# caki35/UNet-Torch

Measured on AMD Instinct MI355X. Metric: images/sec training step, 4-level U-Net 1ch→2cls 512×512, at 1/2/4/8 MI355X, higher is better.
Workload: dtype f16

## Files before the change

### unet-torch_amd/csrc/conv_mfma.hip

```cpp
#include "kernels.h"
#include <stdlib.h>

typedef _Float16 half8 __attribute__((ext_vector_type(8)));
typedef _Float16 half4 __attribute__((ext_vector_type(4)));
typedef float floatx16 __attribute__((ext_vector_type(16)));

#ifdef UMI_STAMP
__device__ unsigned long long umi_stamp_buf[2048 * 8];
#define UMI_T(var)                                                                        \
    unsigned long long var;                                                               \
    __builtin_amdgcn_sched_barrier(0);                                                    \
    asm volatile("s_memtime %0\n\ts_waitcnt lgkmcnt(0)" : "=s"(var)::"memory");           \
    __builtin_amdgcn_sched_barrier(0)
extern "C" int umi_debug_read_stamps(void* dst) {
    return (int)hipMemcpyFromSymbol(dst, HIP_SYMBOL(umi_stamp_buf), sizeof(umi_stamp_buf));
}
#endif

namespace {

constexpr int HALO_W = 34;
constexpr int ROWB = 48;

template <int TH, int BN, int SC = 1, bool K32 = false>
struct Cfg {
    static_assert(!K32 || SC == 2, "K32 stages 32-channel halo tiles");
    static constexpr int WN = BN / 64;
    static constexpr int WM = 4 / WN;
    static_assert(TH / WM == 4, "every wave owns 4 image rows");
    static constexpr int HALO_PIX = (TH + 2) * HALO_W;
    static constexpr int NQ = 2 * SC;
    static constexpr int HROWB = NQ * 16 + 16;
    static constexpr int HPASS = 256 / NQ;
    static constexpr int HB = HALO_PIX * HROWB;
    static constexpr int WROWB = K32 ? 64 : ROWB;
    static constexpr int WSTG = 3 * BN * 64;
    static constexpr int WB = K32 ? 2 * WSTG : 9 * BN * ROWB;
    static constexpr int P = TH * 32;
    static constexpr int ERS = BN * 2 + 16;
    static constexpr int EB = P * ERS;
    static constexpr int SMEM = (HB + WB) > EB ? (HB + WB) : EB;
    static constexpr int KPH = (HALO_PIX + HPASS - 1) / HPASS;
    static constexpr int NPW = K32 ? 3 * BN * 4 : 9 * BN * 2;
    static constexpr int KPW = (NPW + 255) / 256;
    static constexpr int TSTEP = 128 / BN;
    static constexpr bool W_LAST_PARTIAL = !K32 && (KPW - 1) * TSTEP + (TSTEP - 1) >= 9;
    static constexpr int WCO = BN / 32, WRW = 4 / WCO;
    static_assert(!K32 || TH == 8 * WRW, "K32: every wave owns 8 image rows");
    static constexpr int PRE = SC == 2 ? 6 : 8;
};

struct BnRed { const half_t* y; int ld; const float4* tx; const float* rstd; };

__device__ __forceinline__ void* umi_uniform_ptr(const void* p) {
    const unsigned long a = (unsigned long)p;
    const unsigned lo = __builtin_amdgcn_readfirstlane((unsigned)a), hi = __builtin_amdgcn_readfirstlane((unsigned)(a >> 32));
    return (void*)(((unsigned long)hi << 32) | lo);
}

struct Tile { int n, ty0, tx0, c0, cvalid, pt; };

template <int TH, int BN, int SC, bool K32, bool HAS_TX, int EPI>
__global__ __launch_bounds__(256, 2) void conv3x3_mfma_kernel(
    const half_t* __restrict__ x, int ldx, const float4* __restrict__ tx, const half_t* __restrict__ wp8,
    half_t* __restrict__ y, int ldy, float* __restrict__ part, int N, int H, int W, int Ci, int Co, int tiles_x,
    int tiles_y, int n_co, int xcd_chunk, BnRed bn) {
    using C = Cfg<TH, BN, SC, K32>;
    constexpr int HROWB = C::HROWB;
    __shared__ __attribute__((aligned(16))) unsigned char smem[C::SMEM];
    __shared__ float4 txbuf[2][16 * SC];

    const int tid = threadIdx.x;
    const int lane = tid & 63;
    const int wave = tid >> 6;
    const int wn = wave % C::WN, wm = wave / C::WN;
#ifdef UMI_STAMP
    UMI_T(t_start);
    unsigned long long seg[5] = {0, 0, 0, 0, 0}, t_epi = 0, t_pro = 0, eps[4] = {0, 0, 0, 0};
    unsigned n_chunks_done = 0;
#endif

    const int q = (tid >> 3) & 1;
    const int srow = ((tid >> 4) << 3) | (tid & 7);
    const int hq = SC == 1 ? q : (tid >> 3) & (C::NQ - 1);
    const int hrow = SC == 1 ? srow : ((tid >> 5) << 3) | (tid & 7);

    const int tap0 = srow / BN, wcol = srow % BN;
    const int Ci8 = Ci >> 3;
    const int wstep_s = __builtin_amdgcn_readfirstlane(C::TSTEP * Ci8 * Co * 16);
    const int wl_base = C::HB + srow * ROWB + q * 16;
    const bool w_last_ok = tap0 + (C::KPW - 1) * C::TSTEP < 9;
    const int wl_last = w_last_ok ? wl_base + (C::KPW - 1) * 128 * ROWB : C::HB + srow * ROWB + 32;

    const int lrow = lane & 31, lhalf = lane >> 5;
    const int b_base = ((wm * 4) * HALO_W + lrow) * HROWB + lhalf * 16;
    const int a_base = C::HB + (wn * 64 + lrow) * ROWB + lhalf * 16;
    const int wc = wave % C::WCO, wr = wave / C::WCO;
    const int l16 = lane & 15, lg = lane >> 4;
    const int bk_base = ((wr * 8) * HALO_W + l16) * HROWB + lg * 16;
    const int ak_base = C::HB + (wc * 32 + l16) * C::WROWB + ((lg ^ ((l16 >> 1) & 3)) * 16);
    const int wkl_base = C::HB + (((tid >> 5) << 3) | (tid & 7)) * C::WROWB + ((((tid >> 3) & 3) ^ ((tid >> 1) & 3)) * 16);
    const int wdy_s = __builtin_amdgcn_readfirstlane(3 * Ci8 * Co * 16);
    const int nchunks = Ci >> 4;

    constexpr unsigned OOB = 0x7FFFFFFFu;
    constexpr unsigned WBAD = 0x40000000u;
    unsigned hoff[C::KPH];
    int hl_a, hl_b, hl_last;
    unsigned wbase_v, wbase_l;
    __amdgpu_buffer_rsrc_t xrs, wrs;

    auto decode = [&](int item) {
        int wid = item;
        if (xcd_chunk > 0 && wid < 8 * xcd_chunk) wid = (wid & 7) * xcd_chunk + (wid >> 3);
        Tile t;
        const int cb = wid % n_co;
        t.pt = wid / n_co;
        t.n = t.pt / (tiles_x * tiles_y);
        const int rem = t.pt - t.n * tiles_x * tiles_y;
        t.ty0 = (rem / tiles_x) * TH;
        t.tx0 = (rem % tiles_x) * 32;
        t.c0 = cb * BN;
        t.cvalid = Co - t.c0 < BN ? Co - t.c0 : BN;
        return t;
    };
#define UMI_PLAN(t_)                                                                                                   \
    do {                                                                                                              \
        int tid_ = threadIdx.x;                                                                                       \
        asm volatile("" : "+v"(tid_));                                                                                \
        const int q = (tid_ >> 3) & 1, srow = ((tid_ >> 4) << 3) | (tid_ & 7);                                        \
        const int hq = SC == 1 ? q : (tid_ >> 3) & (C::NQ - 1), hrow = SC == 1 ? srow : ((tid_ >> 5) << 3) | (tid_ & 7); \
        const int tap0 = srow / BN, wcol = srow % BN;                                                                 \
        const unsigned wbase = (unsigned)(((tap0 * (Ci >> 3) + q) * Co + wcol) * 16);                                 \
        const bool w_last_ok = tap0 + (C::KPW - 1) * C::TSTEP < 9;                                                    \
        _Pragma("unroll") for (int k = 0; k < C::KPH; ++k) {                                                          \
                                 \
            const int hp = hrow + C::HPASS * k;                                                                       \
            const int hy = hp / HALO_W, hx = hp - hy * HALO_W;                                                        \
            const int gy = (t_).ty0 + hy - 1, gx = (t_).tx0 + hx - 1;                                                 \
            const bool inimg = (hp < C::HALO_PIX) && gy >= 0 && gy < H && gx >= 0 && gx < W;                          \
            hoff[k] = inimg ? (unsigned)(gy * W + gx) * (unsigned)(ldx * 2) + hq * 16 : OOB;                          \
            const int hpc = hp < C::HALO_PIX ? hp : C::HALO_PIX - 1;                                                  \
            if (k == C::KPH - 1) hl_last = inimg ? hp * HROWB + hq * 16 : hpc * HROWB + C::NQ * 16;                   \
        }                                                                                                             \
        hl_a = hrow * HROWB + hq * 16;                                                                                \
        hl_b = hrow * HROWB + C::NQ * 16;                                                                             \
        xrs = __builtin_amdgcn_make_buffer_rsrc(umi_uniform_ptr(x + (long)(t_).n * H * W * ldx), 0,                   \
                                                (int)((long)H * W * ldx * 2), 0x00020000);                            \
        wrs = __builtin_amdgcn_make_buffer_rsrc(umi_uniform_ptr(wp8 + (long)(t_).c0 * 8), 0,                          \
                                                (int)((long)9 * Ci * Co * 2 - (long)(t_).c0 * 16), 0x00020000);       \
        const bool wok = wcol < (t_).cvalid;                                   \
        wbase_v = wok ? wbase : WBAD;                                                                                 \
        wbase_l = (wok && w_last_ok) ? wbase : WBAD;                                                                  \
        if constexpr (K32) {        \
            const int wrow_ = ((tid_ >> 5) << 3) | (tid_ & 7), wq_ = (tid_ >> 3) & 3;                                 \
            const unsigned wb_ = (unsigned)((wq_ * Co + wrow_) * 16);                                                 \
            wbase_v = wrow_ < (t_).cvalid ? wb_ : WBAD;                                                               \
            wbase_l = wrow_ + 64 < (t_).cvalid ? wb_ + 64 * 16 : WBAD;                                                \
        }                                                                                                             \
    } while (0)
#define UMI_ZERO_PADDING()                                                                                             \
    do {                                                                                                              \
        int tid_ = threadIdx.x;                                                                                       \
        asm volatile("" : "+v"(tid_));                                                                                \
        const int hq = SC == 1 ? (tid_ >> 3) & 1 : (tid_ >> 3) & (C::NQ - 1);                                         \
        const int hrow = SC == 1 ? ((tid_ >> 4) << 3) | (tid_ & 7) : ((tid_ >> 5) << 3) | (tid_ & 7);                 \
        _Pragma("unroll") for (int k = 0; k < C::KPH; ++k) {                                                          \
            const int hp = hrow + C::HPASS * k;                                                                       \
            if (hp < C::HALO_PIX && hoff[k] == OOB) {                                                                 \
                unsigned z0 = 0;                                                                                      \
                asm volatile("" : "+v"(z0));         \
                *reinterpret_cast<uint4*>(smem + hp * HROWB + hq * 16) = make_uint4(z0, z0, z0, z0);                  \
            }                                                                                                         \
        }                                                                                                             \
    } while (0)

    half8 hraw[C::KPH], wraw[C::KPW];
#define UMI_ISSUE_H(sc_)                                                                                          \
    do {                                                                                                          \
        _Pragma("unroll") for (int k = 0; k < C::KPH; ++k)                                                        \
            hraw[k] = __builtin_bit_cast(half8, __builtin_amdgcn_raw_buffer_load_b128(xrs, hoff[k], (sc_) * (32 * SC), 0)); \
    } while (0)
#define UMI_ISSUE_W(c_)                                                                                           \
    do {                                                                                                          \
        _Pragma("unroll") for (int k = 0; k < C::KPW; ++k)                                                        \
            wraw[k] = __builtin_bit_cast(half8, __builtin_amdgcn_raw_buffer_load_b128(                            \
                wrs, (C::W_LAST_PARTIAL && k == C::KPW - 1) ? wbase_l : wbase_v, (c_) * 2 * Co * 16 + k * wstep_s, 0)); \
    } while (0)

#define UMI_ISSUE_WK(sc_, dx_)                                                                                    \
    do {                                                                                                          \
        const int ws_ = (((dx_) * Ci8 + 4 * (sc_)) * Co) * 16;                                                    \
        _Pragma("unroll") for (int k = 0; k < C::KPW; ++k)                                                        \
            wraw[k] = __builtin_bit_cast(half8, __builtin_amdgcn_raw_buffer_load_b128(                            \
                wrs, (BN == 128 && (k & 1)) ? wbase_l : wbase_v, ws_ + (BN == 128 ? k >> 1 : k) * wdy_s, 0));     \
    } while (0)

    const bool tx_wave = __builtin_amdgcn_readfirstlane(tid >> 6) == 0;
    const int txi = lane & (16 * SC - 1);
    const int txs = (txi & 7) * C::NQ + (txi >> 3);
    const int nsc = nchunks / SC;
    float4 txr = make_float4(0.f, 1.f, 0.f, 0.f);
    int txc = 0;
    const __amdgpu_buffer_rsrc_t txrs = __builtin_amdgcn_make_buffer_rsrc(umi_uniform_ptr(tx), 0, HAS_TX ? Ci * 16 : 0, 0x00020000);
#define UMI_TX_ROWS(sc_) __builtin_bit_cast(float4, __builtin_amdgcn_raw_buffer_load_b128(txrs, txi * 16, (sc_) * (16 * SC * 16), 0))

    const Tile cur = decode(blockIdx.x);
    UMI_PLAN(cur);
    UMI_ISSUE_H(0);
    half8 wraw1[K32 ? C::KPW : 1];
    if constexpr (K32) {
        UMI_ISSUE_WK(0, 0);
#pragma unroll
        for (int k = 0; k < C::KPW; ++k)
            wraw1[k] = __builtin_bit_cast(half8, __builtin_amdgcn_raw_buffer_load_b128(
                wrs, (BN == 128 && (k & 1)) ? wbase_l : wbase_v, Ci8 * Co * 16 + (BN == 128 ? k >> 1 : k) * wdy_s, 0));
    } else UMI_ISSUE_W(0);
    UMI_ZERO_PADDING();
    if (HAS_TX) {
        if (tx_wave) {
            txbuf[0][txs] = UMI_TX_ROWS(0);
            txbuf[1][txs] = UMI_TX_ROWS(1 % nsc);
            txc = 2 % nsc;
            txr = UMI_TX_ROWS(txc);
        }
        __syncthreads();
    }
    {
        typedef float floatx4 __attribute__((ext_vector_type(4)));
        floatx16 acc[2][4];
        floatx4 acck[2][16];
        if constexpr (K32) {
#pragma unroll
            for (int a = 0; a < 2; ++a)
#pragma unroll
                for (int b = 0; b < 16; ++b)
#pragma unroll
                    for (int r = 0; r < 4; ++r) acck[a][b][r] = 0.f;
        } else {
#pragma unroll
            for (int a = 0; a < 2; ++a)
#pragma unroll
                for (int b = 0; b < 4; ++b)
#pragma unroll
                    for (int r = 0; r < 16; ++r) acc[a][b][r] = 0.f;
        }
#ifdef UMI_STAMP
        UMI_T(t_loop);
        if (n_chunks_done == 0) t_pro = t_loop - t_start;
#endif
        if constexpr (!K32) {
        for (int ci_ = 0; ci_ < nchunks; ++ci_) {
            const int sci = ci_ / SC, sub = ci_ % SC;
            const bool first = SC == 1 || sub == 0;
#ifdef UMI_STAMP
            UMI_T(t0);
            asm volatile("s_waitcnt vmcnt(0)" ::: "memory");
            UMI_T(t0b);
#endif
            if (first) {
                if (HAS_TX) {
                    float4 t[8];
#pragma unroll
                    for (int j = 0; j < 8; ++j) t[j] = txbuf[sci & 1][j * C::NQ + hq];
#pragma unroll
                    for (int k = 0; k < C::KPH; ++k) hraw[k] = umi_tx8(hraw[k], t);
                }
#pragma unroll
                for (int k = 0; k < C::KPH; ++k)
                    *reinterpret_cast<half8*>(smem + (k == C::KPH - 1 ? hl_last : (hoff[k] != OOB ? hl_a : hl_b) + k * C::HPASS * HROWB)) = hraw[k];
            }
#pragma unroll
            for (int k = 0; k < C::KPW; ++k)
                *reinterpret_cast<half8*>(smem + ((C::W_LAST_PARTIAL && k == C::KPW - 1) ? wl_last : wl_base + k * 128 * ROWB)) = wraw[k];
#ifdef UMI_STAMP
            UMI_T(t1);
#endif
            __syncthreads();
#ifdef UMI_STAMP
            UMI_T(t2);
#endif
            if (first) {
                if (HAS_TX && tx_wave) {
                    txbuf[sci & 1][txs] = txr;
                    txc = txc + 1 < nsc ? txc + 1 : 0;
                    txr = UMI_TX_ROWS(txc);
                }
                if (sci + 1 < nsc) UMI_ISSUE_H(sci + 1);
            }
            if (ci_ + 1 < nchunks) UMI_ISSUE_W(ci_ + 1);

            __builtin_amdgcn_s_setprio(3);
#pragma unroll
            for (int dx = 0; dx < 3; ++dx) {
                half8 bf[6];
#pragma unroll
                for (int rr = 0; rr < 6; ++rr)
                    bf[rr] = *reinterpret_cast<const half8*>(smem + b_base + (rr * HALO_W + dx) * HROWB + sub * 32);
#pragma unroll
                for (int dy = 0; dy < 3; ++dy) {
                    half8 af[2];
#pragma unroll
                    for (int mt = 0; mt < 2; ++mt)
                        af[mt] = *reinterpret_cast<const half8*>(smem + a_base + ((dy * 3 + dx) * BN + mt * 32) * ROWB);
#pragma unroll
                    for (int mt = 0; mt < 2; ++mt)
#pragma unroll
                        for (int nt = 0; nt < 4; ++nt)
                            acc[mt][nt] = __builtin_amdgcn_mfma_f32_32x32x16_f16(af[mt], bf[nt + dy], acc[mt][nt], 0, 0, 0);
                }
            }
            constexpr int MPR = 2;
            __builtin_amdgcn_sched_group_barrier(0x100, C::PRE, 0);
#pragma unroll
            for (int i_ = 0; i_ < 36 - C::PRE; ++i_) {
                __builtin_amdgcn_sched_group_barrier(0x008, MPR, 0);
                __builtin_amdgcn_sched_group_barrier(0x100, 1, 0);
            }
            __builtin_amdgcn_sched_group_barrier(0x008, 36 * MPR - MPR * (36 - C::PRE), 0);
            __builtin_amdgcn_s_setprio(0);
#ifdef UMI_STAMP
            UMI_T(t3);
#endif
            __syncthreads();
#ifdef UMI_STAMP
            UMI_T(t4);
            seg[0] += t0b - t0; seg[1] += t1 - t0b; seg[2] += t2 - t1; seg[3] += t3 - t2; seg[4] += t4 - t3;
            ++n_chunks_done;
#endif
        }
        } else {
#pragma unroll
        for (int k = 0; k < C::KPW; ++k) *reinterpret_cast<half8*>(smem + wkl_base + k * 64 * C::WROWB) = wraw[k];
#pragma unroll
        for (int k = 0; k < C::KPW; ++k) wraw[k] = wraw1[k];
        int sci = 0, dx = 0, wcur = 0;
        const int nst = 3 * nsc;
        for (int st = 0; st < nst; ++st) {
            const bool first = dx == 0;
#ifdef UMI_STAMP
            UMI_T(t0);
            asm volatile("s_waitcnt vmcnt(0)" ::: "memory");
            UMI_T(t0b);
#endif
            if (first) {
#ifndef UMI_X_NOTX
                if (HAS_TX) {
                    float4 t[8];
#pragma unroll
                    for (int j = 0; j < 8; ++j) t[j] = txbuf[sci & 1][j * C::NQ + hq];
#pragma unroll
                    for (int k = 0; k < C::KPH; ++k) hraw[k] = umi_tx8(hraw[k], t);
                }
#endif
#ifdef UMI_X_NOHW
#pragma unroll
                for (int k = 0; k < C::KPH; ++k) asm volatile("" ::"v"(hraw[k]));
#else
#pragma unroll
                for (int k = 0; k < C::KPH; ++k)
                    *reinterpret_cast<half8*>(smem + (k == C::KPH - 1 ? hl_last : (hoff[k] != OOB ? hl_a : hl_b) + k * C::HPASS * HROWB)) = hraw[k];
#endif
            }
#ifdef UMI_STAMP
            UMI_T(t1);
#endif
            if (first) __syncthreads();
#ifdef UMI_STAMP
            UMI_T(t2);
#endif
            if (first) {
                if (HAS_TX && tx_wave) {
                    txbuf[sci & 1][txs] = txr;
                    txc = txc + 1 < nsc ? txc + 1 : 0;
                    txr = UMI_TX_ROWS(txc);
                }
                if (sci + 1 < nsc) UMI_ISSUE_H(sci + 1);
            }
            __builtin_amdgcn_s_setprio(3);
            {
                half8 af[3][2];
                const unsigned char* ap = smem + ak_base + wcur;
#pragma unroll
                for (int dy = 0; dy < 3; ++dy)
#pragma unroll
                    for (int ct = 0; ct < 2; ++ct)
                        af[dy][ct] = *reinterpret_cast<const half8*>(ap + (dy * BN + ct * 16) * C::WROWB);
                const unsigned char* bp = smem + bk_base + dx * HROWB;
#pragma unroll
                for (int hr = 0; hr < 10; ++hr)
#pragma unroll
                    for (int h = 0; h < 2; ++h) {
                        const half8 bf = *reinterpret_cast<const half8*>(bp + (hr * HALO_W + h * 16) * HROWB);
#pragma unroll
                        for (int dy = 0; dy < 3; ++dy) {
                            const int r = hr - dy;
                            if (r >= 0 && r < 8) {
#pragma unroll
                                for (int ct = 0; ct < 2; ++ct)
                                    acck[ct][r * 2 + h] = __builtin_amdgcn_mfma_f32_16x16x32_f16(af[dy][ct], bf, acck[ct][r * 2 + h], 0, 0, 0);
                            }
                        }
                    }
            }
            {
#ifdef UMI_X_NOWWRITE
#pragma unroll
                for (int k = 0; k < C::KPW; ++k) asm volatile("" ::"v"(wraw[k]));
#else
#pragma unroll
                for (int k = 0; k < C::KPW; ++k)
                    *reinterpret_cast<half8*>(smem + wkl_base + (C::WSTG - wcur) + k * 64 * C::WROWB) = wraw[k];
#endif
#ifndef UMI_X_NOWLOAD
                const int ndx = dx == 0 ? 2 : dx - 1;
                int nsci = dx == 0 ? sci : sci + 1;
                nsci = nsci < nsc ? nsci : nsc - 1;
                UMI_ISSUE_WK(nsci, ndx);
#endif
            }
#define UMI_G(n_) __builtin_amdgcn_sched_group_barrier(0x008, n_, 0); __builtin_amdgcn_sched_group_barrier(0x100, 1, 0)
            __builtin_amdgcn_sched_group_barrier(0x100, 10, 0);
            UMI_G(2); UMI_G(2); UMI_G(4); UMI_G(4);
            UMI_G(6); UMI_G(6); UMI_G(6); UMI_G(6); UMI_G(6); UMI_G(6); UMI_G(6); UMI_G(6); UMI_G(6); UMI_G(6); UMI_G(6); UMI_G(6);
#pragma unroll
            for (int i_ = 0; i_ < C::KPW; ++i_) {
                __builtin_amdgcn_sched_group_barrier(0x008, 1, 0);
                __builtin_amdgcn_sched_group_barrier(0x200, 1, 0);
            }
#pragma unroll
            for (int i_ = 0; i_ < C::KPW; ++i_) {
                __builtin_amdgcn_sched_group_barrier(0x008, (12 - C::KPW) / C::KPW, 0);
                __builtin_amdgcn_sched_group_barrier(0x020, 1, 0);
            }
#undef UMI_G
            __builtin_amdgcn_s_setprio(0);
#ifdef UMI_STAMP
            UMI_T(t3);
#endif
            __syncthreads();
#ifdef UMI_STAMP
            UMI_T(t4);
            seg[0] += t0b - t0; seg[1] += t1 - t0b; seg[2] += t2 - t1; seg[3] += t3 - t2; seg[4] += t4 - t3;
            ++n_chunks_done;
#endif
            wcur = C::WSTG - wcur;
            if (++dx == 3) { dx = 0; ++sci; }
        }
        }
#ifdef UMI_STAMP
        UMI_T(t_ep0);
#endif

        const int n = cur.n, ty0 = cur.ty0, tx0 = cur.tx0, c0 = cur.c0, cvalid = cur.cvalid, pt = cur.pt;
        if constexpr (K32) {
#pragma unroll
            for (int ct = 0; ct < 2; ++ct) {
                const int co = wc * 32 + ct * 16 + lg * 4;
                float4 ot[4];
                if (EPI == 3) {
#pragma unroll
                    for (int j = 0; j < 4; ++j)
                        ot[j] = co + j < cvalid ? bn.tx[c0 + co + j] : make_float4(0.f, 1.f, 0.f, 0.f);
                }
#pragma unroll
                for (int pt_ = 0; pt_ < 16; ++pt_) {
                    const int pix = (wr * 8 + (pt_ >> 1)) * 32 + (pt_ & 1) * 16 + l16;
                    half4 h;
#pragma unroll
                    for (int j = 0; j < 4; ++j) {
                        float v = acck[ct][pt_][j];
                        if (EPI == 3) v = umi_tx(v, ot[j]);
                        h[j] = (half_t)v;
                    }
                    *reinterpret_cast<half4*>(smem + pix * C::ERS + co * 2) = h;
                }
            }
        } else
#pragma unroll
        for (int mt = 0; mt < 2; ++mt)
#pragma unroll
            for (int g = 0; g < 4; ++g) {
                const int co = wn * 64 + mt * 32 + g * 8 + lhalf * 4;
                float4 ot[4];
                if (EPI == 3) {
#pragma unroll
                    for (int j = 0; j < 4; ++j)
                        ot[j] = co + j < cvalid ? bn.tx[c0 + co + j] : make_float4(0.f, 1.f, 0.f, 0.f);
                }
#pragma unroll
                for (int nt = 0; nt < 4; ++nt) {
                    const int pix = (wm * 4 + nt) * 32 + lrow;
                    half4 h;
#pragma unroll
                    for (int j = 0; j < 4; ++j) {
                        float v = acc[mt][nt][g * 4 + j];
                        if (EPI == 3) v = umi_tx(v, ot[j]);
                        h[j] = (half_t)v;
                    }
                    *reinterpret_cast<half4*>(smem + pix * C::ERS + co * 2) = h;
                }
            }
        __syncthreads();
#ifdef UMI_STAMP
        UMI_T(t_e1);
        eps[0] += t_e1 - t_ep0;
#endif

        constexpr int PPR = BN / 8;
        constexpr int PSTEP = 256 / PPR;
        constexpr int NK = C::P / PSTEP;
        const bool full_tile = (ty0 + TH <= H) && (tx0 + 32 <= W);
        constexpr int SL = PSTEP;
        const int cg = tid % PPR, sl = tid / PPR;
        float s[8], s2[8];
#pragma unroll
        for (int jj = 0; jj < 8; ++jj) s[jj] = s2[jj] = 0.f;
        {
            const int j = cg, p0 = sl;
            const unsigned char* sbase = smem + p0 * C::ERS + j * 16;
            const bool col_ok = j * 8 < cvalid;
            float4 t[8];
            float rs_[8];
            if (EPI == 2 && col_ok) {
#pragma unroll
                for (int jj = 0; jj < 8; ++jj) { t[jj] = bn.tx[c0 + j * 8 + jj]; rs_[jj] = bn.rstd[c0 + j * 8 + jj]; }
            }
#define UMI_EPI_REDUCE(v_, yv_)                                                                                        \
            do {                                                                                                      \
                if (EPI == 1) {                                                                                       \
                    const half8 hv = __builtin_bit_cast(half8, v_);                                                   \
                    _Pragma("unroll") for (int jj = 0; jj < 8; ++jj) { float f = (float)hv[jj]; s[jj] += f; s2[jj] = fmaf(f, f, s2[jj]); } \
                } else if (EPI == 2) {                                                                                \
                    const half8 hv = __builtin_bit_cast(half8, v_);                                                   \
                    _Pragma("unroll") for (int jj = 0; jj < 8; ++jj) {                                                \
                        const float yy = (float)(yv_)[jj];                                                            \
                        const float dz = umi_tx_pre(yy, t[jj]) > t[jj].w ? (float)hv[jj] : 0.f;                       \
                        s[jj] += dz;                                                                                  \
                        s2[jj] = fmaf(dz, (yy - t[jj].x) * rs_[jj], s2[jj]);                                          \
                    }                                                                                                 \
                }                                                                                                     \
            } while (0)
            const bool whole = __builtin_amdgcn_readfirstlane((int)(full_tile && cvalid == BN)) != 0;
            const long tile_pix = ((long)n * H + ty0) * W + tx0;
            half_t* ybase = y + tile_pix * ldy + c0 + j * 8;
            half8 yv[NK];
            if (EPI == 2 && whole) {
                const __amdgpu_buffer_rsrc_t brs = __builtin_amdgcn_make_buffer_rsrc(umi_uniform_ptr(bn.y + tile_pix * bn.ld + c0), 0, 0x7FFFF000, 0x00020000);
                const unsigned bvo = (unsigned)(p0 * bn.ld + j * 8) * 2u;
#pragma unroll
                for (int k = 0; k < NK; ++k)
                    yv[k] = __builtin_bit_cast(half8, __builtin_amdgcn_raw_buffer_load_b128(
                        brs, bvo, ((((k * PSTEP) >> 5) * W + ((k * PSTEP) & 31)) * bn.ld) * 2, 0));
            }
#ifdef UMI_STAMP
            UMI_T(t_e2);
            eps[1] += t_e2 - t_e1;
#endif
            if (whole) {
                const __amdgpu_buffer_rsrc_t yrs = __builtin_amdgcn_make_buffer_rsrc(umi_uniform_ptr(y + tile_pix * ldy + c0), 0, 0x7FFFF000, 0x00020000);
                const unsigned yvo = (unsigned)(p0 * ldy + j * 8) * 2u;
#pragma unroll
                for (int k = 0; k < NK; ++k) {
                    const uint4 v = *reinterpret_cast<const uint4*>(sbase + k * PSTEP * C::ERS);
                    typedef unsigned u32x4_t __attribute__((__vector_size__(4 * sizeof(unsigned))));
                    const u32x4_t vv = __builtin_bit_cast(u32x4_t, v);
                    __builtin_amdgcn_raw_buffer_store_b128(vv, yrs, yvo, ((((k * PSTEP) >> 5) * W + ((k * PSTEP) & 31)) * ldy) * 2, 0);
                    asm volatile("s_nop 1" ::"v"(vv));
                    UMI_EPI_REDUCE(v, yv[k]);
                }
            } else {
                const half_t* yb = EPI == 2 ? bn.y + tile_pix * bn.ld + c0 + j * 8 : nullptr;
#pragma unroll 8
                for (int k = 0; k < NK; ++k) {
                    const int p = p0 + k * PSTEP;
                    const int row = p >> 5, col = p & 31;
                    if (col_ok && (full_tile || (ty0 + row < H && tx0 + col < W))) {
                        const uint4 v = *reinterpret_cast<const uint4*>(sbase + k * PSTEP * C::ERS);
                        *reinterpret_cast<uint4*>(ybase + ((long)row * W + col) * ldy) = v;
                        half8 yv1;
                        if (EPI == 2) yv1 = *reinterpret_cast<const half8*>(yb + ((long)row * W + col) * bn.ld);
                        UMI_EPI_REDUCE(v, yv1);
                    }
                }
            }
#undef UMI_EPI_REDUCE
#ifdef UMI_STAMP
            UMI_T(t_e3);
            eps[2] += t_e3 - t_e2;
#endif
        }

        if (EPI == 1 || EPI == 2) {
            __syncthreads();
            float* rs = reinterpret_cast<float*>(smem);
#pragma unroll
            for (int j = 0; j < 8; ++j) {
                rs[(0 * SL + sl) * BN + cg * 8 + j] = s[j];
                rs[(1 * SL + sl) * BN + cg * 8 + j] = s2[j];
            }
            __syncthreads();
            if (tid < 2 * BN) {
                const int which = tid / BN, cc = tid % BN;
                float a = 0.f;
#pragma unroll 8
                for (int k = 0; k < SL; ++k) a += rs[(which * SL + k) * BN + cc];
                if (cc < cvalid) part[((long)pt * 2 + which) * Co + c0 + cc] = a;
            }
        }
#ifdef UMI_STAMP
        UMI_T(t_end);
        t_epi += t_end - t_ep0;
#endif
    }
#ifdef UMI_STAMP
    if (lane == 0 && blockIdx.x < 512) {
#pragma unroll
        for (int i = 0; i < 5; ++i) umi_stamp_buf[(blockIdx.x * 4 + wave) * 8 + i] = seg[i];
        umi_stamp_buf[(blockIdx.x * 4 + wave) * 8 + 5] = n_chunks_done;
        umi_stamp_buf[(blockIdx.x * 4 + wave) * 8 + 6] = t_pro;
#ifdef UMI_STAMP_EPI
        for (int i = 0; i < 3; ++i) umi_stamp_buf[(blockIdx.x * 4 + wave) * 8 + i] = eps[i];
#endif
        umi_stamp_buf[(blockIdx.x * 4 + wave) * 8 + 7] = t_epi * (unsigned long long)nchunks / (n_chunks_done ? n_chunks_done : 1);
    }
#endif
}

template <int TH, int BN, int SC, bool K32 = false>
int launch(const void* x, int ldx, const void* tx, const void* wp8, void* y, int ldy, float* part, int N, int H, int W,
           int Ci, int Co, const BnRed* bnred, hipStream_t s, const void* out_tx = nullptr) {
    const int tiles_x = (W + 31) / 32, tiles_y = (H + TH - 1) / TH, n_co = (Co + BN - 1) / BN;
    const long nblk = (long)N * tiles_x * tiles_y * n_co;
    if (nblk >= (1L << 31)) return UMI_ERR_UNSUPPORTED;
    dim3 grid((unsigned)nblk), block(256);
    static const bool xcd_off = [] { const char* e = getenv("UMI_CONV_NO_XCD_ORDER"); return e && e[0] == '1'; }();
    const int xcd_chunk = (n_co > 1 && !xcd_off) ? (int)(nblk / 8) : 0;
    const BnRed bn = bnred ? *bnred : BnRed{nullptr, 0, (const float4*)out_tx, nullptr};
#define GO(HT, EP)                                                                                               \
    hipLaunchKernelGGL((conv3x3_mfma_kernel<TH, BN, SC, K32, HT, EP>), grid, block, 0, s, (const half_t*)x, ldx, \
                       (const float4*)tx, (const half_t*)wp8, (half_t*)y, ldy, part, N, H, W, Ci, Co, tiles_x,   \
                       tiles_y, n_co, xcd_chunk, bn)
    if (out_tx) { if (tx) GO(true, 3); else GO(false, 3); }
    else if (bnred) { if (tx) GO(true, 2); else GO(false, 2); }
    else if (tx) { if (part) GO(true, 1); else GO(true, 0); }
    else    { if (part) GO(false, 1); else GO(false, 0); }
#undef GO
    UMI_LAUNCH_CHECK();
    return UMI_OK;
}

#undef UMI_ISSUE_H
#undef UMI_TX_ROWS
#undef UMI_ISSUE_W
#undef UMI_ISSUE_WK
#undef UMI_PLAN
#undef UMI_ZERO_PADDING
}

bool umi_conv3x3_mfma_ok(const ConvFwdProblem& p) {
    if (p.flags & (UMI_CONV_UPSAMPLE2 | UMI_CONV_FORCE_GENERIC)) return false;
    if (p.in_dtype != UMI_F16 || p.out_dtype != UMI_F16 || p.has_bias) return false;
    if (p.R != 3 || p.S != 3 || p.stride != 1 || p.pad != 1 || p.Ho != p.H || p.Wo != p.W) return false;
    if (p.Ci % 16 || p.Co % 8 || p.ldx % 8 || p.ldy % 8) return false;
    if ((long)p.N * p.H * p.W * (long)(p.ldx > p.ldy ? p.ldx : p.ldy) >= (1L << 40)) return false;
    return true;
}

#ifdef UMI_FORCE_BN64
static bool use_bn128(int Co) { (void)Co; return false; }
#else
static bool use_bn128(int Co) { return Co % 128 == 0; }
#endif

static int g_impl = [] { const char* e = getenv("UMI_CONV3X3_IMPL"); return e ? atoi(e) : 1; }();
extern "C" int umi_tune_conv3x3_impl(int impl) {
    const int old = g_impl;
    if (impl >= 1 && impl <= 8) g_impl = impl;
    return old;
}

static int pick_th(int Co) { return use_bn128(Co) ? 8 : 16; }

int umi_conv3x3_mfma_stat_rows(int N, int H, int W, int Co) {
    const int th = pick_th(Co);
    return N * ((W + 31) / 32) * ((H + th - 1) / th);
}

#define UMI_GO(x, tx, wp8, y, part, ...)                                                     \
    do {                                                                                     \
        const int Ci = p.Ci, Co = p.Co;                                                      \
        if (use_bn128(Co) && Ci % 32 == 0 && g_impl != 2)                                    \
            return launch<8, 128, 2, true>(x, p.ldx, tx, wp8, y, p.ldy, part, p.N, p.H, p.W, Ci, Co, __VA_ARGS__); \
        if (use_bn128(Co)) return launch<8, 128, 1>(x, p.ldx, tx, wp8, y, p.ldy, part, p.N, p.H, p.W, Ci, Co, __VA_ARGS__); \
        if (Ci % 32 == 0 && g_impl == 3)                                                     \
            return launch<16, 64, 2, true>(x, p.ldx, tx, wp8, y, p.ldy, part, p.N, p.H, p.W, Ci, Co, __VA_ARGS__); \
        if (Ci % 32 == 0 && g_impl != 2)                                                     \
            return launch<16, 64, 2>(x, p.ldx, tx, wp8, y, p.ldy, part, p.N, p.H, p.W, Ci, Co, __VA_ARGS__); \
        return launch<16, 64, 1>(x, p.ldx, tx, wp8, y, p.ldy, part, p.N, p.H, p.W, Ci, Co, __VA_ARGS__); \
    } while (0)

int umi_conv3x3_mfma(const ConvFwdProblem& p, const void* x, const void* tx, const void* wp8, void* y, float* stat_part,
                     hipStream_t s) {
    UMI_GO(x, tx, wp8, y, stat_part, nullptr, s);
}

int umi_conv3x3_mfma_bnred(const ConvFwdProblem& p, const void* dy, const void* wp8, void* da, const void* ybn, int ldybn,
                           const void* txbn, const float* rstd, float* part, hipStream_t s) {
    const BnRed bn{(const half_t*)ybn, ldybn, (const float4*)txbn, rstd};
    UMI_GO(dy, nullptr, wp8, da, part, &bn, s);
}

int umi_conv3x3_mfma_act(const ConvFwdProblem& p, const void* x, const void* tx, const void* wp8, const void* out_tx, void* y,
                         hipStream_t s) {
    UMI_GO(x, tx, wp8, y, nullptr, nullptr, s, out_tx);
}
#undef UMI_GO
```

Baseline: 748.3.

## Prefetch epilogue bn.y residual tile into idle halo/weight registers during final K steps

For the fused BN-reduce epilogue (EPI==2) in the K32 conv path, the kernel now reuses the halo and weight prefetch registers. Once the last input chunk and the final weight loads are no longer needed, it loads the bn.y tile pieces into them early. The epilogue then takes those pieces from registers instead of issuing fresh global loads after the main loop. The aim is to hide epilogue load latency behind the last MFMA steps. The cost is extra control logic and index arithmetic in the hot loop, which may raise register pressure or disturb the scheduler groupings.

After: 749.3, median of 4. No clear change (+0.1%).

```diff
diff --git a/unet-torch_amd/csrc/conv_mfma.hip b/unet-torch_amd/csrc/conv_mfma.hip
--- a/unet-torch_amd/csrc/conv_mfma.hip
+++ b/unet-torch_amd/csrc/conv_mfma.hip
@@ -206,6 +206,30 @@
 #define UMI_TX_ROWS(sc_) __builtin_bit_cast(float4, __builtin_amdgcn_raw_buffer_load_b128(txrs, txi * 16, (sc_) * (16 * SC * 16), 0))
 
     const Tile cur = decode(blockIdx.x);
+    constexpr bool YPRE = EPI == 2 && K32;
+    const bool ywhole = YPRE && __builtin_amdgcn_readfirstlane(
+        (int)(cur.ty0 + TH <= H && cur.tx0 + 32 <= W && cur.cvalid == BN)) != 0;
+    constexpr int EPPR = BN / 8, EPSTEP = 256 / EPPR, ENK = C::P / EPSTEP;
+    constexpr int YH = !YPRE ? 0 : (C::KPH < ENK ? C::KPH : ENK);
+    constexpr int YW = !YPRE ? 0 : (C::KPW < ENK - YH ? C::KPW : ENK - YH);
+#define UMI_Y_RSRC()                                                                                               \
+    __builtin_amdgcn_make_buffer_rsrc(umi_uniform_ptr(bn.y + (((long)cur.n * H + cur.ty0) * W + cur.tx0) * bn.ld + cur.c0), 0, \
+                                      0x7FFFF000, 0x00020000)
+#define UMI_Y_SOFF(k_) (((((k_) * EPSTEP) >> 5) * W + (((k_) * EPSTEP) & 31)) * bn.ld * 2)
+#define UMI_Y_VOFF(var_)                                                                                           \
+    unsigned var_;                                                                                                \
+    do {                                                                                                          \
+        int tid_ = threadIdx.x;                                                                                   \
+        asm volatile("" : "+v"(tid_));                                                                            \
+        var_ = (unsigned)((tid_ / EPPR) * bn.ld + (tid_ % EPPR) * 8) * 2u;                                        \
+    } while (0)
+#define UMI_ISSUE_YH()                                                                                             \
+    do {                                                                                                          \
+        const __amdgpu_buffer_rsrc_t brs_ = UMI_Y_RSRC();                                                         \
+        UMI_Y_VOFF(bvo_);                                                                                         \
+        _Pragma("unroll") for (int k = 0; k < YH; ++k)                                                            \
+            hraw[k] = __builtin_bit_cast(half8, __builtin_amdgcn_raw_buffer_load_b128(brs_, bvo_, UMI_Y_SOFF(k), 0)); \
+    } while (0)
     UMI_PLAN(cur);
     UMI_ISSUE_H(0);
     half8 wraw1[K32 ? C::KPW : 1];
@@ -336,8 +360,21 @@
         for (int k = 0; k < C::KPW; ++k) wraw[k] = wraw1[k];
         int sci = 0, dx = 0, wcur = 0;
         const int nst = 3 * nsc;
+        __amdgpu_buffer_rsrc_t yw_rs = wrs;
+        unsigned yw_v = wbase_v, yw_l = wbase_l;
+        int yw_co = Co, yw_sb = 0, yw_step = wdy_s;
         for (int st = 0; st < nst; ++st) {
             const bool first = dx == 0;
+            if (YPRE && ywhole && st == nst - 2) {
+                static_assert(!YPRE || (YW == C::KPW && (BN != 128 || YH % 2 == 0)), "wraw[] carries whole rows of bn.y pieces");
+                yw_rs = UMI_Y_RSRC();
+                UMI_Y_VOFF(bvo_);
+                yw_v = bvo_;
+                yw_l = bvo_ + 16 * bn.ld * 2;
+                yw_co = 0;
+                yw_sb = UMI_Y_SOFF(YH);
+                yw_step = W * bn.ld * 2;
+            }
 #ifdef UMI_STAMP
             UMI_T(t0);
             asm volatile("s_waitcnt vmcnt(0)" ::: "memory");
@@ -376,6 +413,7 @@
                     txr = UMI_TX_ROWS(txc);
                 }
                 if (sci + 1 < nsc) UMI_ISSUE_H(sci + 1);
+                else if (YPRE && ywhole) UMI_ISSUE_YH();
             }
             __builtin_amdgcn_s_setprio(3);
             {
@@ -416,6 +454,13 @@
                 const int ndx = dx == 0 ? 2 : dx - 1;
                 int nsci = dx == 0 ? sci : sci + 1;
                 nsci = nsci < nsc ? nsci : nsc - 1;
+                if constexpr (YPRE) {
+                    const int ws_ = ((ndx * Ci8 + 4 * nsci) * yw_co) * 16 + yw_sb;
+#pragma unroll
+                    for (int k = 0; k < C::KPW; ++k)
+                        wraw[k] = __builtin_bit_cast(half8, __builtin_amdgcn_raw_buffer_load_b128(
+                            yw_rs, (BN == 128 && (k & 1)) ? yw_l : yw_v, ws_ + (BN == 128 ? k >> 1 : k) * yw_step, 0));
+                } else
                 UMI_ISSUE_WK(nsci, ndx);
 #endif
             }
@@ -541,17 +586,21 @@
                     }                                                                                                 \
                 }                                                                                                     \
             } while (0)
-            const bool whole = __builtin_amdgcn_readfirstlane((int)(full_tile && cvalid == BN)) != 0;
+            const bool whole = YPRE ? ywhole : __builtin_amdgcn_readfirstlane((int)(full_tile && cvalid == BN)) != 0;
             const long tile_pix = ((long)n * H + ty0) * W + tx0;
             half_t* ybase = y + tile_pix * ldy + c0 + j * 8;
+            static_assert(EPPR == PPR && EPSTEP == PSTEP && ENK == NK, "the prefetch uses the epilogue's piece mapping");
             half8 yv[NK];
             if (EPI == 2 && whole) {
                 const __amdgpu_buffer_rsrc_t brs = __builtin_amdgcn_make_buffer_rsrc(umi_uniform_ptr(bn.y + tile_pix * bn.ld + c0), 0, 0x7FFFF000, 0x00020000);
                 const unsigned bvo = (unsigned)(p0 * bn.ld + j * 8) * 2u;
 #pragma unroll
-                for (int k = 0; k < NK; ++k)
-                    yv[k] = __builtin_bit_cast(half8, __builtin_amdgcn_raw_buffer_load_b128(
+                for (int k = 0; k < NK; ++k) {
+                    if (k < YH) yv[k] = hraw[k < YH ? k : 0];
+                    else if (k < YH + YW) yv[k] = wraw[k >= YH && k < YH + YW ? k - YH : 0];
+                    else yv[k] = __builtin_bit_cast(half8, __builtin_amdgcn_raw_buffer_load_b128(
                         brs, bvo, ((((k * PSTEP) >> 5) * W + ((k * PSTEP) & 31)) * bn.ld) * 2, 0));
+                }
             }
 #ifdef UMI_STAMP
             UMI_T(t_e2);
@@ -651,6 +700,10 @@
 }
 
 #undef UMI_ISSUE_H
+#undef UMI_ISSUE_YH
+#undef UMI_Y_RSRC
+#undef UMI_Y_SOFF
+#undef UMI_Y_VOFF
 #undef UMI_TX_ROWS
 #undef UMI_ISSUE_W
 #undef UMI_ISSUE_WK
```
